# zc402/video-classification

Measured on AMD Instinct MI355X. Metric: clips/sec SlowFast-R50 8x8, 32x224^2 bf16 training step, higher is better.
Workload: dtype bf16

## Files before the change

video-classification_amd/build.py:

```python
import os
import subprocess
from concurrent.futures import ThreadPoolExecutor

HERE = os.path.dirname(os.path.abspath(__file__))
ROOT = os.path.dirname(HERE)
CSRC = os.path.join(HERE, "csrc")
LIB = os.path.join(HERE, "libsfk.so")
SOURCES = ["conv_igemm.hip", "conv_igemm_p8.hip", "conv_halo.hip", "conv_pw.hip", "conv_wgrad.hip", "conv_wgrad_p8.hip", "conv_wgrad_band.hip", "stem_conv.hip", "bn.hip", "bn_tail.hip", "pool_head.hip",
           "optim_misc.hip", "eval_input.hip", "stem2d.hip", "roi_resize.hip", "sgd.hip"]


def _newer(a, b):
    return (not os.path.exists(b)) or os.path.getmtime(a) > os.path.getmtime(b)


def build(force: bool = False, verbose: bool = False) -> str:
    hipcc = os.environ.get("HIPCC", "/opt/rocm/bin/hipcc")
    if not os.path.exists(hipcc):
        hipcc = "hipcc"
    objdir = os.path.join(HERE, "build")
    os.makedirs(objdir, exist_ok=True)
    deps = [os.path.join(CSRC, "sfk_common.h"), os.path.join(CSRC, "conv_igemm_epi.h"), os.path.join(CSRC, "conv_wgrad_common.h"), os.path.join(CSRC, "conv_wgrad_band_acc.inc"), os.path.join(ROOT, "include", "sfk.h"),
            os.path.join(ROOT, "include", "sfk_stem2d.h"), os.path.join(ROOT, "include", "sfk_u8stem.h"),
            os.path.join(ROOT, "include", "sfk_v2.h")]
    flags = ["--offload-arch=gfx950", "-O3", "-fPIC", "-std=c++17", "-I" + os.path.join(ROOT, "include"), "-I" + CSRC]
    flags += os.environ.get("SFK_EXTRA_FLAGS", "").split()

    def compile_one(src):
        s = os.path.join(CSRC, src)
        o = os.path.join(objdir, src.replace(".hip", ".o"))
        if force or _newer(s, o) or any(_newer(d, o) for d in deps):
            cmd = [hipcc] + flags + ["-c", s, "-o", o]
            if verbose:
                print(" ".join(cmd))
            subprocess.run(cmd, check=True)
            return o, True
        return o, False

    with ThreadPoolExecutor(max_workers=min(4, len(SOURCES))) as ex:
        res = list(ex.map(compile_one, SOURCES))
    objs = [o for o, _ in res]
    if force or any(ch for _, ch in res) or not os.path.exists(LIB):
        subprocess.run([hipcc, "--offload-arch=gfx950", "-shared", "-fPIC", "-o", LIB] + objs, check=True)
    return LIB


if __name__ == "__main__":
    print(build(force="--force" in os.sys.argv, verbose=True))
```

video-classification_amd/csrc/conv_halo.hip:

```cpp
#include "conv_igemm_epi.h"

namespace sfk_igemm {

typedef __attribute__((address_space(3))) void lds_void_h_t;

struct HaloTaps { int widx[9]; };

template <int EPI>
__global__ __launch_bounds__(256, 1) void conv_halo_kernel(const ConvK k, const HaloTaps ht, const int nbands, const int bands_per_frame) {
  using T = bf16_t;
  constexpr int C = 64, W = 56;
  constexpr int R = 4;
  constexpr int PW = 64;
  constexpr int PB = C * 2;
  constexpr int ROWBYTES = PW * PB;
  constexpr int BAND = (R + 2) * ROWBYTES;
  constexpr int NBI = BAND / 1024 / 4;
  constexpr int NK = 18;
  constexpr int BM = R * W;
  constexpr int RED0 = 2 * BAND;
  constexpr uint32_t FAR = 0x80000000u;
  __shared__ __attribute__((aligned(16))) char smem[RED0 + 2048];

  const int tid = threadIdx.x, lane = tid & 63;
  const int wave = __builtin_amdgcn_readfirstlane(tid >> 6);
  const int wm = wave & 1, wn = wave >> 1;
  const int l15 = lane & 15, g4 = lane >> 4;
  const int b0 = (gridDim.x & 7) == 0 ? (int)((blockIdx.x & 7) * (gridDim.x >> 3) + (blockIdx.x >> 3)) : (int)blockIdx.x;
  if (b0 >= nbands) return;
  const __amdgpu_buffer_rsrc_t xrs = sfk_make_rsrc(k.x, k.xbytes);
  auto fsw = [](int q) { return ((q >> 1) & 3) << 1; };

  uint32_t bsrc[NBI];
#pragma unroll
  for (int ii = 0; ii < NBI; ++ii) {
    const int qd = (wave * NBI + ii) * 8 + (lane >> 3);
    const int ri = qd / PW, wi = qd % PW;
    const int ls = (lane & 7) ^ fsw(qd);
    bsrc[ii] = (wi >= 1 && wi <= W) ? (uint32_t)((ri * W + wi) * k.xld * 2 + k.xoff * 2 + ls * 16) : FAR;
  }
  int nb_base = 0, nb_r0 = 0;
  auto band_begin = [&](const int b_) __attribute__((always_inline)) {
    const int b = b_ < nbands ? b_ : 0;
    const int fr = b / bands_per_frame;
    nb_r0 = (b - fr * bands_per_frame) * R;
    nb_base = ((fr * k.xh + nb_r0) * W - W - 1) * k.xld * 2;
  };
  auto issue_band = [&](const int buf, const int first, const int count) __attribute__((always_inline)) {
    char* dst = smem + buf * BAND + wave * NBI * 1024;
#pragma unroll
    for (int ii = first; ii < first + count; ++ii) {
      const int ri = (wave * NBI + ii) * 8 / PW;
      const bool rok = (unsigned)(nb_r0 - 1 + ri) < (unsigned)k.xh;
      const uint32_t vo = (rok && bsrc[ii] != FAR) ? (uint32_t)((int)bsrc[ii] + nb_base) : FAR;
      __builtin_amdgcn_raw_ptr_buffer_load_lds(xrs, (lds_void_h_t*)(dst + ii * 1024), 16, (int)vo, 0, 0, 0);
    }
  };
  band_begin(b0);
  issue_band(0, 0, NBI);

  bf16x8 wreg[2][NK];
  {
    const bf16_t* wp = static_cast<const bf16_t*>(k.w);
#pragma unroll
    for (int i = 0; i < 2; ++i) {
      const int co = wn * 32 + 16 * i + l15;
#pragma unroll
      for (int n = 0; n < NK; ++n)
        wreg[i][n] = *reinterpret_cast<const bf16x8*>(wp + ((int64_t)co * k.wtaps + ht.widx[n >> 1]) * k.cin + 32 * (n & 1) + 8 * g4);
    }
  }
  uint32_t xa[2][3][7][2];
#pragma unroll
  for (int j = 0; j < 7; ++j) {
    const int p = wm * 112 + 16 * j + l15;
    const int q0 = (p / W) * PW + (p % W) + 1;
#pragma unroll
    for (int dw = 0; dw < 3; ++dw) {
      const int q = q0 + dw - 1;
#pragma unroll
      for (int sk = 0; sk < 2; ++sk)
#pragma unroll
        for (int bf = 0; bf < 2; ++bf) xa[bf][dw][j][sk] = (uint32_t)(bf * BAND + q * PB + (((4 * sk + g4) ^ fsw(q)) << 4));
    }
  }

  f32x4 acc[2][7];
  bf16x8 xfr[2][7];
  constexpr int BPK = 2, BKS = NBI / BPK;
  static_assert(NBI % BPK == 0 && BKS <= NK, "band pieces");

  auto band_body = [&](const int buf, const int b, const bool first) __attribute__((always_inline)) {
    auto rd_x = [&](const int set, const int n) __attribute__((always_inline)) {
      const int tap = n >> 1, dh = tap / 3 - 1, dw = tap % 3;
#pragma unroll
      for (int j = 0; j < 7; ++j) xfr[set][j] = *reinterpret_cast<const bf16x8*>(smem + xa[buf][dw][j][n & 1] + (dh + 1) * ROWBYTES);
    };
#pragma unroll
    for (int i = 0; i < 2; ++i)
#pragma unroll
      for (int j = 0; j < 7; ++j) acc[i][j] = f32x4{0.f, 0.f, 0.f, 0.f};
    band_begin(b + (int)gridDim.x);
    if (first) asm volatile("s_waitcnt vmcnt(0)" ::: "memory");
    __builtin_amdgcn_s_barrier();
    asm volatile("" ::: "memory");
    rd_x(0, 0);
#pragma unroll
    for (int n = 0; n < NK; ++n) {
      if (n < BKS) issue_band(buf ^ 1, n * BPK, BPK);
      if (n + 1 < NK) rd_x((n + 1) & 1, n + 1);
#pragma unroll
      for (int i = 0; i < 2; ++i)
#pragma unroll
        for (int j = 0; j < 7; ++j)
          asm volatile("v_mfma_f32_16x16x32_bf16 %0, %1, %2, %0" : "+a"(acc[i][j]) : "a"(wreg[i][n]), "v"(xfr[n & 1][j]));
    }
    asm volatile("s_waitcnt vmcnt(0)\n\ts_nop 15\n\ts_nop 7" ::: "memory");
    if (k.stats) {
      float* red = reinterpret_cast<float*>(smem + RED0);
#pragma unroll
      for (int i = 0; i < 2; ++i)
#pragma unroll
        for (int r = 0; r < 4; ++r) {
          float s1 = 0.f, s2 = 0.f;
#pragma unroll
          for (int j = 0; j < 7; ++j) {
            const float v = acc[i][j][r];
            s1 += v;
            s2 += v * v;
          }
          s1 = row16_sum(s1);
          s2 = row16_sum(s2);
          if (l15 == 15) {
            const int col = wn * 32 + 16 * i + 4 * g4 + r;
            red[(wm * 64 + col) * 2 + 0] = s1;
            red[(wm * 64 + col) * 2 + 1] = s2;
          }
        }
      __builtin_amdgcn_s_waitcnt(0xC07F);
      __builtin_amdgcn_s_barrier();
      asm volatile("" ::: "memory");
      if (tid < 64) {
        float* o = k.stats + ((int64_t)b * k.cout + tid) * 2;
        o[0] = red[tid * 2 + 0] + red[(64 + tid) * 2 + 0];
        o[1] = red[tid * 2 + 1] + red[(64 + tid) * 2 + 1];
      }
    }
    ConvK ks = k;
    ks.stats = nullptr;
    epilogue_plain<T, EPI, 7, 2, BM, C, 2, 2, true>(ks, acc, nullptr, b, 0, wm, wn, lane, tid);
  };
  for (int b = b0;;) {
    band_body(0, b, b == b0);
    b += gridDim.x;
    if (b >= nbands) break;
    band_body(1, b, false);
    b += gridDim.x;
    if (b >= nbands) break;
  }
}

__attribute__((visibility("hidden"))) bool halo_ok(const sfk_conv_desc* d) {
  if (!sfk_tune().igemm_halo || d->x.dtype != SFK_BF16) return false;
  if (d->cin != 64 || d->cout != 64 || d->x.w != 56) return false;
  if (d->x.h % 4 != 0 || d->x.t != d->y.t || d->x.h != d->y.h || d->x.w != d->y.w || d->rt != d->y.t || d->rh != d->y.h || d->rw != d->y.w)
    return false;
  for (int a = 0; a < 3; ++a)
    if (d->gs[a] != 1 || d->os[a] != 1 || d->oo[a] != 0) return false;
  if (d->ntaps != 9) return false;
  int seen = 0;
  for (int i = 0; i < 9; ++i) {
    if (d->taps[i].dt != 0 || d->taps[i].dh < -1 || d->taps[i].dh > 1 || d->taps[i].dw < -1 || d->taps[i].dw > 1) return false;
    seen |= 1 << ((d->taps[i].dh + 1) * 3 + d->taps[i].dw + 1);
  }
  if (seen != 0x1FF) return false;
  if (d->ep.scale || d->ep.shift || d->bnb.partials || d->out_relu_bits || d->accumulate) return false;
  if ((d->y.ld % 8) || (d->y.c_off % 8) || !sfk_tune().igemm_wide_store) return false;
  return sfk_fmap_bytes(&d->x) < 0x7FF00000ll;
}

__attribute__((visibility("hidden"))) int halo_mtiles(const sfk_conv_desc* d) { return d->x.n * d->x.t * (d->x.h / 4); }

__attribute__((visibility("hidden"))) int launch_halo(const ConvK& k, const sfk_conv_desc* d, hipStream_t s) {
  const int bpf = d->x.h / 4, nbands = d->x.n * d->x.t * bpf;
  const int grid = nbands < 256 ? nbands : 256;
  HaloTaps ht;
  for (int i = 0; i < 9; ++i) ht.widx[(d->taps[i].dh + 1) * 3 + d->taps[i].dw + 1] = d->taps[i].widx;
  hipLaunchKernelGGL((conv_halo_kernel<0>), dim3((unsigned)grid), dim3(256), 0, s, k, ht, nbands, bpf);
  SFK_CHECK_LAUNCH();
  return SFK_OK;
}

}
```

video-classification_amd/csrc/conv_igemm.hip:

```cpp

#include "conv_igemm_epi.h"

using namespace sfk_igemm;

namespace sfk_igemm {
__attribute__((visibility("hidden"))) int launch_p8(const ConvK& k, int bms, dim3 grid, hipStream_t s);
__attribute__((visibility("hidden"))) bool halo_ok(const sfk_conv_desc* d);
__attribute__((visibility("hidden"))) int halo_mtiles(const sfk_conv_desc* d);
__attribute__((visibility("hidden"))) int launch_halo(const ConvK& k, const sfk_conv_desc* d, hipStream_t s);
}

namespace {

template <typename T, int BM, int BN, int WM, int WN, bool SHORTK, int EPI = 0>
__global__ __launch_bounds__(256, (sizeof(T) == 2 ? 3 : 1)) void conv_igemm_kernel(const ConvK k) {
  using TL = Tile<T>;
  constexpr int VEC = TL::VEC, SEGS = TL::SEGS, ROWB = TL::ROWB;
  constexpr int FM = BM / WM / 16, FN = BN / WN / 16;
  constexpr int RPI = 256 / SEGS;
  constexpr int XL = BM / RPI;
  constexpr int WL = (BN + RPI - 1) / RPI;
  constexpr int BUF = (BM + BN) * ROWB;
  static_assert(WM * WN == 4 && BM % RPI == 0, "tile shape");
  __shared__ __attribute__((aligned(16))) char smem[2 * BUF];
  __shared__ sfk_tap s_taps[SFK_MAX_TAPS + 1];
  __shared__ int s_xdelta[SFK_MAX_TAPS + 1];
  __shared__ int s_woff[SFK_MAX_TAPS + 1];
  if (threadIdx.x <= SFK_MAX_TAPS) {
    sfk_tap t = k.taps[threadIdx.x < SFK_MAX_TAPS ? threadIdx.x : 0];
    if ((int)threadIdx.x >= k.ntaps) { t.dt = -128; t.dh = 0; t.dw = 0; t.widx = 0; }
    s_taps[threadIdx.x] = t;
    s_xdelta[threadIdx.x] = (((int)t.dt * k.xh + (int)t.dh) * k.xw + (int)t.dw) * k.xld * (int)sizeof(T);
    s_woff[threadIdx.x] = (int)t.widx * k.cin * (int)sizeof(T);
  }
  __syncthreads();

  const int tid = threadIdx.x, lane = tid & 63, wave = tid >> 6;
  const int wm = wave % WM, wn = wave / WM;
  const int l15 = lane & 15, g = lane >> 4;

  int mt, nt;
  {
    const int nblk = gridDim.x, b = blockIdx.x;
    const int q = nblk >> 3, r = nblk & 7, xcd = b & 7;
    const int logical = (xcd < r ? xcd * (q + 1) : r * (q + 1) + (xcd - r) * q) + (b >> 3);
    nt = logical % k.ntiles;
    mt = logical / k.ntiles;
  }

  const int seg = tid % SEGS, row0 = tid / SEGS;
  int xtb[XL], xhb[XL], xwb[XL];
  uint32_t xbase[XL];
#pragma unroll
  for (int i = 0; i < XL; ++i) {
    const int m = mt * BM + row0 + i * RPI;
    uint32_t q1, rw_, q2, rh_, n_, rt_;
    k.drw.divmod((uint32_t)m, q1, rw_);
    k.drh.divmod(q1, q2, rh_);
    k.drt.divmod(q2, n_, rt_);
    xtb[i] = (m < k.M) ? (int)rt_ * k.gst : -(1 << 28);
    xhb[i] = (int)rh_ * k.gsh;
    xwb[i] = (int)rw_ * k.gsw;
    xbase[i] = (uint32_t)((((((int64_t)n_ * k.xt + (int)rt_ * k.gst) * k.xh + xhb[i]) * k.xw + xwb[i]) * k.xld + k.xoff) *
                          (int64_t)sizeof(T));
  }
  uint32_t wbase[WL];
#pragma unroll
  for (int i = 0; i < WL; ++i) {
    const int r = row0 + i * RPI;
    const int co = nt * BN + r;
    wbase[i] = (r < BN && co < k.cout) ? (uint32_t)(co * k.wtaps * k.cin) * (uint32_t)sizeof(T) : SFK_OOB;
  }
  const __amdgpu_buffer_rsrc_t xrs = sfk_make_rsrc(k.x, k.xbytes);
  const __amdgpu_buffer_rsrc_t wrs = sfk_make_rsrc(k.w, k.wbytes);

  struct Stage { uint4 x[XL]; uint4 w[WL]; };
  auto gload = [&](int step, Stage& st) {
    const uint32_t q = (uint32_t)(step * SEGS + seg);
    uint32_t tap, cseg;
    k.dspt.divmod(q, tap, cseg);
    const bool cok = tap < (uint32_t)k.ntaps;
    const int ti_ = cok ? (int)tap : SFK_MAX_TAPS;
    const sfk_tap tp = s_taps[ti_];
    const uint32_t xd = (uint32_t)(s_xdelta[ti_] + (int)cseg * 16);
    const uint32_t wd = (uint32_t)(s_woff[ti_] + (int)cseg * 16);
#pragma unroll
    for (int i = 0; i < XL; ++i) {
      const int ti = xtb[i] + tp.dt, hi = xhb[i] + tp.dh, wi = xwb[i] + tp.dw;
      const bool ok = cok && (unsigned)ti < (unsigned)k.xt && (unsigned)hi < (unsigned)k.xh &&
                      (unsigned)wi < (unsigned)k.xw;
      st.x[i] = sfk_buffer_load16(xrs, ok ? xbase[i] + xd : SFK_OOB);
    }
#pragma unroll
    for (int i = 0; i < WL; ++i)
      st.w[i] = sfk_buffer_load16(wrs, (cok && wbase[i] != SFK_OOB) ? wbase[i] + wd : SFK_OOB);
  };
  auto lstore = [&](int buf, const Stage& st) {
    char* xs = smem + buf * BUF;
    char* ws = xs + BM * ROWB;
#pragma unroll
    for (int i = 0; i < XL; ++i) *reinterpret_cast<uint4*>(xs + TL::off(row0 + i * RPI, seg)) = st.x[i];
#pragma unroll
    for (int i = 0; i < WL; ++i) {
      const int r = row0 + i * RPI;
      if ((BN % RPI == 0) || r < BN) *reinterpret_cast<uint4*>(ws + TL::off(r, seg)) = st.w[i];
    }
  };

  f32x4 acc[FN][FM];
#pragma unroll
  for (int i = 0; i < FN; ++i)
#pragma unroll
    for (int j = 0; j < FM; ++j) acc[i][j] = f32x4{0.f, 0.f, 0.f, 0.f};

  auto compute = [&](int buf) {
    const char* xs = smem + buf * BUF;
    const char* ws = xs + BM * ROWB;
    typename TL::frag a[FN], b[FM];
#pragma unroll
    for (int i = 0; i < FN; ++i) a[i] = TL::load(ws, wn * (BN / WN) + 16 * i + l15, g);
#pragma unroll
    for (int j = 0; j < FM; ++j) b[j] = TL::load(xs, wm * (BM / WM) + 16 * j + l15, g);
#pragma unroll
    for (int i = 0; i < FN; ++i)
#pragma unroll
      for (int j = 0; j < FM; ++j) TL::mma(acc[i][j], a[i], b[j]);
  };

  Stage r0, r1;
  if constexpr (SHORTK) {
    gload(0, r0);
    lstore(0, r0);
    if (k.KC > 1) gload(1, r1);
    __syncthreads();
    int it = 0;
    for (; it + 3 < k.KC; it += 2) {
      gload(it + 2, r0);
      compute(0);
      lstore(1, r1);
      __syncthreads();
      gload(it + 3, r1);
      compute(1);
      lstore(0, r0);
      __syncthreads();
    }
    const int rem = k.KC - it;
    if (rem == 1) {
      compute(0);
    } else if (rem == 2) {
      compute(0);
      lstore(1, r1);
      __syncthreads();
      compute(1);
    } else {
      gload(it + 2, r0);
      compute(0);
      lstore(1, r1);
      __syncthreads();
      compute(1);
      lstore(0, r0);
      __syncthreads();
      compute(0);
// ... 305 lines not shown
      (d->rw - 1) * d->os[2] + d->oo[2] >= d->y.w)
    return SFK_ERR_INVALID;
  if ((int64_t)d->x.n * d->rt * d->rh * d->rw >= (1ll << 31)) return SFK_ERR_UNSUPPORTED;
  if (!sfk_fmap_vec_ok(&d->x)) return SFK_ERR_UNSUPPORTED;
  if ((d->y.c % 4) || (d->y.ld % 4) || (d->y.c_off % 4) || (((uintptr_t)d->y.ptr) & 15)) return SFK_ERR_UNSUPPORTED;
  if (((uintptr_t)d->w) & 15) return SFK_ERR_UNSUPPORTED;
  const bool bnb_bits = d->bnb.partials && !d->bnb.y_bn.ptr;
  if (d->out_relu_bits) {
    if (d->bnb.partials && !bnb_bits) return SFK_ERR_INVALID;
    if (!relu_out_ok(d)) return SFK_ERR_UNSUPPORTED;
  }
  if (ep_on(d)) {
    const sfk_conv_epilogue& e = d->ep;
    if (d->stats || d->bnb.partials || d->out_relu_bits) return SFK_ERR_INVALID;
    if ((e.relu_bits && !e.relu) || (e.res_scale && !e.res.ptr) || (e.res_shift && !e.res.ptr)) return SFK_ERR_INVALID;
    if (e.res.ptr && (!sfk_fmap_ok(&e.res) || e.res.n != d->y.n || e.res.t != d->y.t || e.res.h != d->y.h ||
                      e.res.w != d->y.w || e.res.c != d->y.c || e.res.dtype != d->y.dtype))
      return SFK_ERR_INVALID;
    if (!lin_out_of(d)) return SFK_ERR_UNSUPPORTED;
    if ((((uintptr_t)e.scale) | ((uintptr_t)e.shift) | ((uintptr_t)e.res_scale) | ((uintptr_t)e.res_shift)) & 15)
      return SFK_ERR_UNSUPPORTED;
    if (d->x.dtype == SFK_BF16) {
      if (d->cout > 16 ? !bnb_ok(d) : (e.res.ptr || e.relu)) return SFK_ERR_UNSUPPORTED;
    }
    if (e.res.ptr && !sfk_fmap_vec_ok(&e.res)) return SFK_ERR_UNSUPPORTED;
    if (sfk_fmap_bytes(&d->y) >= (1ll << 32) - 64 || (e.res.ptr && sfk_fmap_bytes(&e.res) >= (1ll << 32) - 64))
      return SFK_ERR_UNSUPPORTED;
  }
  if (d->bnb.partials) {
    if (sfk_fmap_bytes(&d->y) >= (1ll << 32) - 64) return SFK_ERR_UNSUPPORTED;
    if (d->bnb.y_bn.ptr && sfk_fmap_ok(&d->bnb.y_bn) && sfk_fmap_bytes(&d->bnb.y_bn) >= (1ll << 32) - 64) return SFK_ERR_UNSUPPORTED;
    if (d->bnb.mask_src.ptr && sfk_fmap_ok(&d->bnb.mask_src) && sfk_fmap_bytes(&d->bnb.mask_src) >= (1ll << 32) - 64) return SFK_ERR_UNSUPPORTED;
  }
  if (bnb_bits) {
    if (!d->out_relu_bits || d->stats || d->bnb.mask_src.ptr) return SFK_ERR_INVALID;
    if (!bnb_ok(d) || !lin_out_of(d)) return SFK_ERR_UNSUPPORTED;
  } else if (d->bnb.partials) {
    const sfk_bn_bwd_fuse& b = d->bnb;
    if (d->stats || !sfk_fmap_ok(&b.y_bn) || !b.mean || !b.invstd) return SFK_ERR_INVALID;
    if (b.y_bn.n != d->y.n || b.y_bn.t != d->y.t || b.y_bn.h != d->y.h || b.y_bn.w != d->y.w || b.y_bn.c != d->y.c ||
        b.y_bn.dtype != d->y.dtype)
      return SFK_ERR_INVALID;
    if (b.mask_src.ptr && (!sfk_fmap_ok(&b.mask_src) || b.mask_src.n != d->y.n || b.mask_src.t != d->y.t ||
                           b.mask_src.h != d->y.h || b.mask_src.w != d->y.w || b.mask_src.c != d->y.c ||
                           b.mask_src.dtype != d->y.dtype))
      return SFK_ERR_INVALID;
    if (!b.mask_src.ptr && b.relu && (!b.scale || !b.shift)) return SFK_ERR_INVALID;
    if (!bnb_ok(d)) return SFK_ERR_UNSUPPORTED;
    if (!sfk_fmap_vec_ok(&b.y_bn) || (b.mask_src.ptr && !sfk_fmap_vec_ok(&b.mask_src))) return SFK_ERR_UNSUPPORTED;
  }
  const int64_t esz = d->x.dtype == SFK_BF16 ? 2 : 4;
  if (sfk_fmap_bytes(&d->x) >= (1ll << 32) - 64 || (int64_t)d->cout * d->wtaps * d->cin * esz >= (1ll << 32) - 64)
    return SFK_ERR_UNSUPPORTED;
  return SFK_OK;
}

int launch_dma(const ConvK& k, int bm, dim3 grid, hipStream_t s, int bn = 128) {
  if (bn == 256) {
    if (bm == 224) hipLaunchKernelGGL((conv_igemm_dma_kernel<256, 256, 2, 4, 0, 224>), grid, dim3(512), 0, s, k);
    else hipLaunchKernelGGL((conv_igemm_dma_kernel<256, 256, 4, 2>), grid, dim3(512), 0, s, k);
    SFK_CHECK_LAUNCH();
    return SFK_OK;
  }
  if (k.bn_parts) {
    if (k.bn_y == nullptr) hipLaunchKernelGGL((conv_igemm_dma_kernel<128, 128, 2, 2, 5>), grid, dim3(256), 0, s, k);
    else if (k.bn_mask) hipLaunchKernelGGL((conv_igemm_dma_kernel<128, 128, 2, 2, 7>), grid, dim3(256), 0, s, k);
    else if (k.accumulate) hipLaunchKernelGGL((conv_igemm_dma_kernel<128, 128, 2, 2, 6>), grid, dim3(256), 0, s, k);
    else hipLaunchKernelGGL((conv_igemm_dma_kernel<128, 128, 2, 2, 1>), grid, dim3(256), 0, s, k);
    SFK_CHECK_LAUNCH();
    return SFK_OK;
  }
  if (k.ep_on) {
    if (bm == 256) hipLaunchKernelGGL((conv_igemm_dma_kernel<256, 128, 4, 2, 3>), grid, dim3(512), 0, s, k);
    else if (k.ep_res) hipLaunchKernelGGL((conv_igemm_dma_kernel<128, 128, 2, 2, 4>), grid, dim3(256), 0, s, k);
    else hipLaunchKernelGGL((conv_igemm_dma_kernel<128, 128, 2, 2, 3>), grid, dim3(256), 0, s, k);
    SFK_CHECK_LAUNCH();
    return SFK_OK;
  }
  if (k.obits) {
    if (bm == 256) hipLaunchKernelGGL((conv_igemm_dma_kernel<256, 128, 4, 2, 2>), grid, dim3(512), 0, s, k);
    else hipLaunchKernelGGL((conv_igemm_dma_kernel<128, 128, 2, 2, 2>), grid, dim3(256), 0, s, k);
    SFK_CHECK_LAUNCH();
    return SFK_OK;
  }
  if (bm == 256) hipLaunchKernelGGL((conv_igemm_dma_kernel<256, 128, 4, 2>), grid, dim3(512), 0, s, k);
  else hipLaunchKernelGGL((conv_igemm_dma_kernel<128, 128, 2, 2>), grid, dim3(256), 0, s, k);
  SFK_CHECK_LAUNCH();
  return SFK_OK;
}

template <typename T>
int launch(const sfk_conv_desc* d, hipStream_t s) {
  ConvK k;
  k.x = d->x.ptr; k.y = d->y.ptr; k.w = d->w; k.stats = d->stats;
  k.xt = d->x.t; k.xh = d->x.h; k.xw = d->x.w; k.xld = d->x.ld; k.xoff = d->x.c_off;
  k.yt = d->y.t; k.yh = d->y.h; k.yw = d->y.w; k.yld = d->y.ld; k.yoff = d->y.c_off;
  k.M = d->x.n * d->rt * d->rh * d->rw;
  k.drw.set(d->rw); k.drh.set(d->rh); k.drt.set(d->rt);
  k.gst = d->gs[0]; k.gsh = d->gs[1]; k.gsw = d->gs[2];
  k.ost = d->os[0]; k.osh = d->os[1]; k.osw = d->os[2];
  k.oot = d->oo[0]; k.ooh = d->oo[1]; k.oow = d->oo[2];
  k.cin = d->cin; k.cout = d->cout; k.wtaps = d->wtaps; k.ntaps = d->ntaps;
  const int vec = sfk_vec_of(d->x.dtype), segs = BK / vec;
  k.dspt.set(d->cin / vec);
  k.dkct.set(d->cin / 32 > 0 ? d->cin / 32 : 1);
  k.dk64.set(d->ntaps);
  k.KC = (d->ntaps * (d->cin / vec) + segs - 1) / segs;
  k.accumulate = d->accumulate;
  k.obits = d->out_relu_bits;
  k.bn_parts = d->bnb.partials;
  k.bn_y = nullptr; k.bn_mask = nullptr;
  if (k.bn_parts) {
    k.bn_y = d->bnb.y_bn.ptr; k.bn_yld = d->bnb.y_bn.ld; k.bn_yoff = d->bnb.y_bn.c_off;
    k.bn_mask = d->bnb.mask_src.ptr; k.bn_mld = d->bnb.mask_src.ld; k.bn_moff = d->bnb.mask_src.c_off;
    k.bn_relu = d->bnb.relu;
    k.bn_mean = d->bnb.mean; k.bn_invstd = d->bnb.invstd; k.bn_scale = d->bnb.scale; k.bn_shift = d->bnb.shift;
  }
  k.ep_on = ep_on(d) ? 1 : 0;
  k.ep_scale = d->ep.scale; k.ep_shift = d->ep.shift; k.ep_rscale = d->ep.res_scale; k.ep_rshift = d->ep.res_shift;
  k.ep_res = d->ep.res.ptr; k.ep_rld = d->ep.res.ld; k.ep_roff = d->ep.res.c_off;
  k.ep_relu = d->ep.relu; k.ep_bits = d->ep.relu_bits;
  k.ybytes = (uint32_t)sfk_fmap_bytes(&d->y);
  k.ybig = sfk_fmap_bytes(&d->y) >= (1ll << 32) - 64 ? 1 : 0;
  k.ep_rbytes = d->ep.res.ptr ? (uint32_t)sfk_fmap_bytes(&d->ep.res) : 0u;
  k.bn_ybytes = (k.bn_parts && d->bnb.y_bn.ptr) ? (uint32_t)sfk_fmap_bytes(&d->bnb.y_bn) : 0u;
  k.bn_mbytes = (k.bn_parts && d->bnb.mask_src.ptr) ? (uint32_t)sfk_fmap_bytes(&d->bnb.mask_src) : 0u;
  k.obits_bytes = d->out_relu_bits ? (uint32_t)(sfk_fmap_pixels(&d->y) * (d->cout / sfk_vec_of(d->x.dtype))) : 0u;
  k.kshort = sfk_tune().igemm_short_k;
  k.lin_out = lin_out_of(d);
  const int wide_ok = sfk_tune().igemm_wide_store;
  k.wide_store = (wide_ok || k.obits) && (d->cout % 8) == 0 && (d->y.ld % 8) == 0 && (d->y.c_off % 8) == 0;
  k.xbytes = (uint32_t)sfk_fmap_bytes(&d->x);
  k.wbytes = (uint32_t)((int64_t)d->cout * d->wtaps * d->cin * (d->x.dtype == SFK_BF16 ? 2 : 4));
  for (int i = 0; i < SFK_MAX_TAPS; ++i) k.taps[i] = d->taps[i < d->ntaps ? i : 0];
  if constexpr (sizeof(T) == 2) {
    if (k.ep_on && (d->ep.res.ptr || d->ep.relu) && !d->accumulate && sfk_tune().igemm_pw_stream && d->ntaps == 1 &&
        d->taps[0].dt == 0 && d->taps[0].dh == 0 && d->taps[0].dw == 0 && d->gs[0] == 1 && d->gs[1] == 1 && d->gs[2] == 1 &&
        k.lin_out && d->x.t == d->y.t && d->x.h == d->y.h && d->x.w == d->y.w) {
      const int r = sfk_conv_pw_fused(d, s);
      if (r != SFK_ERR_UNSUPPORTED) return r;
    }
    if (pw_dgrad_rows(d) > 0) return sfk_conv_pw_dgrad(d, s);
    if (pw_plain_route(d)) {
      const int r = sfk_conv_pw_fused(d, s);
      if (r != SFK_ERR_UNSUPPORTED) return r;
    }
  }
  if constexpr (sizeof(T) == 2) {
    if (halo_ok(d)) {
      k.mtiles = halo_mtiles(d);
      k.ntiles = 1;
      return launch_halo(k, d, s);
    }
  }
  const TileSel ts = pick_tile(d);
  k.mtiles = (k.M + ts.bm - 1) / ts.bm;
  k.ntiles = (d->cout + ts.bn - 1) / ts.bn;
  const dim3 grid((unsigned)(k.mtiles * k.ntiles)), block(256);
  if (ts.p8) return launch_p8(k, ts.bm, dim3((unsigned)(k.mtiles * k.ntiles)), s);
  if (ts.dma) return launch_dma(k, ts.bm, grid, s, ts.bn);
  if (k.bn_parts) {
    if constexpr (sizeof(T) == 2) {
      if (k.bn_y == nullptr) {
        if (ts.bn == 128) hipLaunchKernelGGL((conv_igemm_kernel<T, 128, 128, 2, 2, false, 5>), grid, block, 0, s, k);
        else if (ts.bn == 64) hipLaunchKernelGGL((conv_igemm_kernel<T, 256, 64, 4, 1, false, 5>), grid, block, 0, s, k);
        else hipLaunchKernelGGL((conv_igemm_kernel<T, 256, 32, 4, 1, false, 5>), grid, block, 0, s, k);
      } else if (k.bn_mask) {
        if (ts.bn == 128) hipLaunchKernelGGL((conv_igemm_kernel<T, 128, 128, 2, 2, false, 7>), grid, block, 0, s, k);
        else if (ts.bn == 64) hipLaunchKernelGGL((conv_igemm_kernel<T, 256, 64, 4, 1, false, 7>), grid, block, 0, s, k);
        else hipLaunchKernelGGL((conv_igemm_kernel<T, 256, 32, 4, 1, false, 7>), grid, block, 0, s, k);
      } else if (k.accumulate) {
        if (ts.bn == 128) hipLaunchKernelGGL((conv_igemm_kernel<T, 128, 128, 2, 2, false, 6>), grid, block, 0, s, k);
        else if (ts.bn == 64) hipLaunchKernelGGL((conv_igemm_kernel<T, 256, 64, 4, 1, false, 6>), grid, block, 0, s, k);
        else hipLaunchKernelGGL((conv_igemm_kernel<T, 256, 32, 4, 1, false, 6>), grid, block, 0, s, k);
      } else if (ts.bn == 128) hipLaunchKernelGGL((conv_igemm_kernel<T, 128, 128, 2, 2, false, 1>), grid, block, 0, s, k);
      else if (ts.bn == 64) hipLaunchKernelGGL((conv_igemm_kernel<T, 256, 64, 4, 1, false, 1>), grid, block, 0, s, k);
      else hipLaunchKernelGGL((conv_igemm_kernel<T, 256, 32, 4, 1, false, 1>), grid, block, 0, s, k);
      SFK_CHECK_LAUNCH();
      return SFK_OK;
    }
    return SFK_ERR_UNSUPPORTED;
  }
  if (k.ep_on) {
    if (ts.bn == 128) hipLaunchKernelGGL((conv_igemm_kernel<T, 128, 128, 2, 2, false, 3>), grid, block, 0, s, k);
    else if (ts.bn == 64) hipLaunchKernelGGL((conv_igemm_kernel<T, 256, 64, 4, 1, false, 3>), grid, block, 0, s, k);
    else if (ts.bn == 32) hipLaunchKernelGGL((conv_igemm_kernel<T, 256, 32, 4, 1, false, 3>), grid, block, 0, s, k);
    else hipLaunchKernelGGL((conv_igemm_kernel<T, 256, 16, 4, 1, false, 3>), grid, block, 0, s, k);
    SFK_CHECK_LAUNCH();
    return SFK_OK;
  }
  if (k.obits) {
    if (ts.bn == 128) hipLaunchKernelGGL((conv_igemm_kernel<T, 128, 128, 2, 2, false, 2>), grid, block, 0, s, k);
    else if (ts.bn == 64) hipLaunchKernelGGL((conv_igemm_kernel<T, 256, 64, 4, 1, false, 2>), grid, block, 0, s, k);
    else if (ts.bn == 32) hipLaunchKernelGGL((conv_igemm_kernel<T, 256, 32, 4, 1, false, 2>), grid, block, 0, s, k);
    else if (sizeof(T) == 4) hipLaunchKernelGGL((conv_igemm_kernel<T, 256, 16, 4, 1, false, 2>), grid, block, 0, s, k);
    else return SFK_ERR_UNSUPPORTED;
    SFK_CHECK_LAUNCH();
    return SFK_OK;
  }
  if (k.KC <= k.kshort && ts.bn <= 32) {
    if (ts.bn == 32) hipLaunchKernelGGL((conv_igemm_kernel<T, 256, 32, 4, 1, true>), grid, block, 0, s, k);
    else hipLaunchKernelGGL((conv_igemm_kernel<T, 256, 16, 4, 1, true>), grid, block, 0, s, k);
  } else {
    if (ts.bn == 128) hipLaunchKernelGGL((conv_igemm_kernel<T, 128, 128, 2, 2, false>), grid, block, 0, s, k);
    else if (ts.bn == 64) hipLaunchKernelGGL((conv_igemm_kernel<T, 256, 64, 4, 1, false>), grid, block, 0, s, k);
    else if (ts.bn == 32) hipLaunchKernelGGL((conv_igemm_kernel<T, 256, 32, 4, 1, false>), grid, block, 0, s, k);
    else hipLaunchKernelGGL((conv_igemm_kernel<T, 256, 16, 4, 1, false>), grid, block, 0, s, k);
  }
  SFK_CHECK_LAUNCH();
  return SFK_OK;
}

}

extern "C" int sfk_conv_igemm_mtiles(const sfk_conv_desc* d) {
  const int st = validate(d);
  if (st != SFK_OK) return st;
  const int rows = pw_dgrad_rows(d);
  if (rows > 0) return rows;
  if (halo_ok(d)) return halo_mtiles(d);
  const int64_t M = (int64_t)d->x.n * d->rt * d->rh * d->rw;
  const int bm = pick_tile(d).bm;
  return (int)((M + bm - 1) / bm);
}

extern "C" int sfk_conv_relu_out_supported(const sfk_conv_desc* d) {
  if (!d || d->struct_size != sizeof(sfk_conv_desc)) return 0;
  sfk_conv_desc c = *d;
  c.out_relu_bits = nullptr;
  if (validate(&c) != SFK_OK) return 0;
  return relu_out_ok(d) ? 1 : 0;
}

extern "C" int sfk_conv_igemm_family(const sfk_conv_desc* d) {
  if (validate(d) != SFK_OK) return -1;
  if (d->x.dtype == SFK_BF16) {
    if (ep_on(d) && (d->ep.res.ptr || d->ep.relu) && !d->accumulate && sfk_tune().igemm_pw_stream && d->ntaps == 1 &&
        d->taps[0].dt == 0 && d->taps[0].dh == 0 && d->taps[0].dw == 0 && d->gs[0] == 1 && d->gs[1] == 1 && d->gs[2] == 1 &&
        lin_out_of(d) && d->x.t == d->y.t && d->x.h == d->y.h && d->x.w == d->y.w && d->cin <= 128 &&
        ((d->cout == 32 || d->cout == 64 || d->cout == 128) ? d->cin <= 32 : (d->cout == 256 ? (d->cin > 32 && d->cin <= 64) : (d->cout == 512 && d->cin > 96))))
      return 3;
    if (pw_dgrad_rows(d) > 0) return 3;
    if (pw_plain_route(d)) return 3;
  }
  if (halo_ok(d)) return 5;
  const TileSel ts = pick_tile(d);
  return ts.p8 ? 4 : (ts.dma ? 1 : 0);
}

extern "C" int sfk_conv_epilogue_supported(const sfk_conv_desc* d) {
  return (d && ep_on(d) && validate(d) == SFK_OK) ? 1 : 0;
}

extern "C" int sfk_conv_bnb_supported(const sfk_conv_desc* d) {
  if (!d || d->struct_size != sizeof(sfk_conv_desc)) return 0;
  sfk_conv_desc c = *d;
  c.bnb.partials = nullptr;
  if (validate(&c) != SFK_OK) return 0;
  return bnb_ok(d) ? 1 : 0;
}

extern "C" int sfk_conv_igemm(const sfk_conv_desc* d, sfk_stream_t stream) {
  const int st = validate(d);
  if (st != SFK_OK) return st;
  hipStream_t s = static_cast<hipStream_t>(stream);
  return d->x.dtype == SFK_BF16 ? launch<bf16_t>(d, s) : launch<float>(d, s);
}
```

video-classification_amd/csrc/optim_misc.hip:

```cpp
#include <string.h>

#include "sfk_common.h"

namespace {

__global__ void adam_step_inc_kernel(int64_t* step) { step[0] += 1; }

template <typename S>
__global__ __launch_bounds__(256) void adam_kernel(float* __restrict__ p, const float* __restrict__ g,
                                                   float* __restrict__ m, float* __restrict__ v, int64_t count,
                                                   float lr, float b1, float b2, float eps, float gscale,
                                                   const int64_t* step, S* __restrict__ shadow) {
  __shared__ float bc[2];
  if (threadIdx.x == 0) {
    const double t = (double)step[0];
    bc[0] = (float)(1.0 - pow((double)b1, t));
    bc[1] = (float)(1.0 - pow((double)b2, t));
  }
  __syncthreads();
  const float step_size = lr / bc[0];
  const float inv_sqrt_bc2 = 1.f / sqrtf(bc[1]);
  for (int64_t i = ((int64_t)blockIdx.x * 256 + threadIdx.x) * 4; i < count; i += (int64_t)gridDim.x * 1024) {
    if (i + 3 < count) {
      float4 pv = *reinterpret_cast<float4*>(p + i);
// ... 18 lines not shown
#pragma unroll
        for (int j = 0; j < 4; ++j) shadow[i + j] = (S)pp[j];
      }
    } else {
      for (int64_t e = i; e < count; ++e) {
        const float gj = g[e] * gscale;
        m[e] = b1 * m[e] + (1.f - b1) * gj;
        v[e] = b2 * v[e] + (1.f - b2) * gj * gj;
        p[e] -= step_size * m[e] / (sqrtf(v[e]) * inv_sqrt_bc2 + eps);
        if (shadow) shadow[e] = (S)p[e];
      }
    }
  }
}

template <typename S, typename D>
__global__ __launch_bounds__(256) void cast_kernel(const S* __restrict__ src, D* __restrict__ dst, int64_t count) {
  for (int64_t i = (int64_t)blockIdx.x * 256 + threadIdx.x; i < count; i += (int64_t)gridDim.x * 256)
    dst[i] = (D)(float)src[i];
}

template <typename S, typename D>
__global__ __launch_bounds__(256) void filter_transpose_kernel(const S* __restrict__ src, D* __restrict__ dst,
                                                               int cout, int wtaps, int cin) {
  const int64_t total = (int64_t)cout * wtaps * cin;
  for (int64_t i = (int64_t)blockIdx.x * 256 + threadIdx.x; i < total; i += (int64_t)gridDim.x * 256) {
    const int co = (int)(i % cout);
    const int64_t r = i / cout;
    const int wi = (int)(r % wtaps);
    const int ci = (int)(r / wtaps);
    dst[i] = (D)(float)src[((int64_t)co * wtaps + wi) * cin + ci];
  }
}

template <typename D>
__global__ __launch_bounds__(256) void filter_refresh_kernel(const float* __restrict__ master, D* __restrict__ s,
                                                             D* __restrict__ st, const sfk_filter_ent* __restrict__ table,
                                                             int n) {
  __shared__ float tile[32][33];
  int lo = 0, hi = n - 1;
  const int b = blockIdx.x;
  while (lo < hi) {
    const int mid = (lo + hi + 1) >> 1;
    if (table[mid].first_block <= b) lo = mid; else hi = mid - 1;
  }
  const sfk_filter_ent e = table[lo];
  const int tiles_ci = (e.cin + 31) / 32;
  int lb = b - e.first_block;
  const int tap = lb % e.wtaps;
  lb /= e.wtaps;
  const int ci0 = (lb % tiles_ci) * 32, co0 = (lb / tiles_ci) * 32;
  const int tx = threadIdx.x & 31, ty = threadIdx.x >> 5;
#pragma unroll
  for (int i = 0; i < 4; ++i) {
    const int co = co0 + ty + 8 * i, ci = ci0 + tx;
    float v = 0.f;
    if (co < e.cout && ci < e.cin) {
      const int64_t idx = e.off + ((int64_t)co * e.wtaps + tap) * e.cin + ci;
      v = master[idx];
      if (s) s[idx] = (D)v;
    }
    tile[ty + 8 * i][tx] = v;
  }
  if (!st || !e.transpose) return;
  __syncthreads();
#pragma unroll
  for (int i = 0; i < 4; ++i) {
    const int ci = ci0 + ty + 8 * i, co = co0 + tx;
    if (co < e.cout && ci < e.cin) st[e.off + ((int64_t)ci * e.wtaps + tap) * e.cout + co] = (D)tile[tx][ty + 8 * i];
  }
}

inline unsigned grid_for(int64_t total, int per_thread = 1) {
  int64_t b = (total + 256ll * per_thread - 1) / (256ll * per_thread);
  if (b > 16384) b = 16384;
  if (b < 1) b = 1;
  return (unsigned)b;
}

}

extern "C" int sfk_adam(float* p, const float* g, float* m, float* v, int64_t count, float lr, float beta1,
                        float beta2, float eps, float grad_scale, int64_t* step, void* shadow,
                        int32_t shadow_dtype, sfk_stream_t stream) {
  if (!p || !g || !m || !v || !step || count <= 0) return SFK_ERR_INVALID;
  if ((((uintptr_t)p) | ((uintptr_t)g) | ((uintptr_t)m) | ((uintptr_t)v)) & 15) return SFK_ERR_UNSUPPORTED;
  hipStream_t s = static_cast<hipStream_t>(stream);
  hipLaunchKernelGGL(adam_step_inc_kernel, dim3(1), dim3(1), 0, s, step);
  const dim3 grid(grid_for(count, 4)), blk(256);
  if (shadow && shadow_dtype == SFK_BF16)
    hipLaunchKernelGGL(adam_kernel<bf16_t>, grid, blk, 0, s, p, g, m, v, count, lr, beta1, beta2, eps, grad_scale, step, static_cast<bf16_t*>(shadow));
  else
    hipLaunchKernelGGL(adam_kernel<float>, grid, blk, 0, s, p, g, m, v, count, lr, beta1, beta2, eps, grad_scale, step, static_cast<float*>(shadow));
  SFK_CHECK_LAUNCH();
  return SFK_OK;
}


static inline bool dtype_ok(int d) { return d == SFK_F32 || d == SFK_BF16; }

extern "C" int sfk_filter_transpose(const void* src, int32_t src_dtype, void* dst, int32_t dst_dtype, int32_t cout,
                                    int32_t wtaps, int32_t cin, sfk_stream_t stream) {
  if (!src || !dst || cout <= 0 || wtaps <= 0 || cin <= 0 || !dtype_ok(src_dtype) || !dtype_ok(dst_dtype))
    return SFK_ERR_INVALID;
  hipStream_t s = static_cast<hipStream_t>(stream);
  const int64_t total = (int64_t)cout * wtaps * cin;
  if (src_dtype == SFK_F32 && dst_dtype == SFK_F32)
    hipLaunchKernelGGL((filter_transpose_kernel<float, float>), dim3(grid_for(total)), dim3(256), 0, s, (const float*)src, (float*)dst, cout, wtaps, cin);
  else if (src_dtype == SFK_F32 && dst_dtype == SFK_BF16)
    hipLaunchKernelGGL((filter_transpose_kernel<float, bf16_t>), dim3(grid_for(total)), dim3(256), 0, s, (const float*)src, (bf16_t*)dst, cout, wtaps, cin);
  else if (src_dtype == SFK_BF16 && dst_dtype == SFK_F32)
    hipLaunchKernelGGL((filter_transpose_kernel<bf16_t, float>), dim3(grid_for(total)), dim3(256), 0, s, (const bf16_t*)src, (float*)dst, cout, wtaps, cin);
  else
    hipLaunchKernelGGL((filter_transpose_kernel<bf16_t, bf16_t>), dim3(grid_for(total)), dim3(256), 0, s, (const bf16_t*)src, (bf16_t*)dst, cout, wtaps, cin);
  SFK_CHECK_LAUNCH();
  return SFK_OK;
}

extern "C" int sfk_filter_refresh(const float* master, void* s, void* st, int32_t dtype, const sfk_filter_ent* table,
                                  int32_t n_layers, int32_t total_blocks, sfk_stream_t stream) {
  if (!master || (!s && !st) || !table || n_layers <= 0 || total_blocks <= 0 || !dtype_ok(dtype)) return SFK_ERR_INVALID;
  hipStream_t hs = static_cast<hipStream_t>(stream);
  if (dtype == SFK_BF16)
    hipLaunchKernelGGL((filter_refresh_kernel<bf16_t>), dim3((unsigned)total_blocks), dim3(256), 0, hs, master, (bf16_t*)s, (bf16_t*)st, table, n_layers);
  else
    hipLaunchKernelGGL((filter_refresh_kernel<float>), dim3((unsigned)total_blocks), dim3(256), 0, hs, master, (float*)s, (float*)st, table, n_layers);
  SFK_CHECK_LAUNCH();
  return SFK_OK;
}

extern "C" int sfk_cast(const void* src, int32_t src_dtype, void* dst, int32_t dst_dtype, int64_t count,
                        sfk_stream_t stream) {
  if (!src || !dst || count <= 0 || !dtype_ok(src_dtype) || !dtype_ok(dst_dtype)) return SFK_ERR_INVALID;
  hipStream_t s = static_cast<hipStream_t>(stream);
  if (src_dtype == SFK_F32 && dst_dtype == SFK_F32)
    hipLaunchKernelGGL((cast_kernel<float, float>), dim3(grid_for(count, 4)), dim3(256), 0, s, (const float*)src, (float*)dst, count);
  else if (src_dtype == SFK_F32 && dst_dtype == SFK_BF16)
    hipLaunchKernelGGL((cast_kernel<float, bf16_t>), dim3(grid_for(count, 4)), dim3(256), 0, s, (const float*)src, (bf16_t*)dst, count);
  else if (src_dtype == SFK_BF16 && dst_dtype == SFK_F32)
    hipLaunchKernelGGL((cast_kernel<bf16_t, float>), dim3(grid_for(count, 4)), dim3(256), 0, s, (const bf16_t*)src, (float*)dst, count);
  else
    hipLaunchKernelGGL((cast_kernel<bf16_t, bf16_t>), dim3(grid_for(count, 4)), dim3(256), 0, s, (const bf16_t*)src, (bf16_t*)dst, count);
  SFK_CHECK_LAUNCH();
  return SFK_OK;
}

extern "C" int sfk_fill_zero(void* p, size_t bytes, sfk_stream_t stream) {
  if (!p) return SFK_ERR_INVALID;
  if (bytes == 0) return SFK_OK;
  return hipMemsetAsync(p, 0, bytes, static_cast<hipStream_t>(stream)) == hipSuccess ? SFK_OK : SFK_ERR_LAUNCH;
}

namespace {
constexpr sfk_tuning kDefaults = {(uint32_t)sizeof(sfk_tuning), 5, 0, 1, 192, 256, 1, 7, 1024, 0, 48, 150, 1, 1ll << 20, 3, 512, 1, 16, 1, 3, 3};
sfk_tuning g_tuning = kDefaults;
bool g_tuning_set = false;
}
const sfk_tuning& sfk_tune() { return g_tuning; }

extern "C" int sfk_default_tuning(sfk_tuning* out) {
  if (!out || out->struct_size != sizeof(sfk_tuning)) return SFK_ERR_INVALID;
  *out = kDefaults;
  return SFK_OK;
}

extern "C" int sfk_get_tuning(sfk_tuning* out) {
  if (!out || out->struct_size != sizeof(sfk_tuning)) return SFK_ERR_INVALID;
  *out = g_tuning;
  return SFK_OK;
}

extern "C" int sfk_init(const sfk_tuning* t) {
  sfk_tuning want = kDefaults;
  if (t) {
    if (t->struct_size != sizeof(sfk_tuning)) return SFK_ERR_INVALID;
    want = *t;
  }
  if (want.bn_parts < 1 || want.wgrad_target_8w < 1 || want.wgrad_target_4w < 1 || want.pool_blocks < 1 ||
      want.igemm_short_k < 0)
    return SFK_ERR_INVALID;
  if (g_tuning_set) return memcmp(&want, &g_tuning, sizeof(want)) == 0 ? SFK_OK : SFK_ERR_INVALID;
  g_tuning = want;
  g_tuning_set = true;
  return SFK_OK;
}

extern "C" int sfk_abi_version(void) { return SFK_ABI_VERSION; }

extern "C" const char* sfk_status_string(int status) {
  switch (status) {
    case SFK_OK: return "ok";
    case SFK_ERR_INVALID: return "invalid argument";
    case SFK_ERR_UNSUPPORTED: return "unsupported shape or alignment";
    case SFK_ERR_LAUNCH: return "kernel launch failed";
    default: return "unknown status";
  }
}
```

Before: 1168.

## Add narrow-channel halo conv kernel for 8- and 16-channel 3x3 convs

Adds a new halo-band implicit-GEMM kernel for small-channel 3x3 spatial convs (8ch at width 56, 16ch at width 28), which in SlowFast are the fast pathway. It packs several taps into one MFMA K-dimension and stages 14-row bands through LDS with double buffering. It also fuses the BN stats reduction into the kernel. The igemm_halo tuning field becomes a bitmask and defaults to enabling both narrow variants, routing these convs away from the generic igemm path, which wastes most of its tile on tiny channel counts. The kernel covers only forward-style convs with no epilogue.

```diff
diff --git a/video-classification_amd/build.py b/video-classification_amd/build.py
--- a/video-classification_amd/build.py
+++ b/video-classification_amd/build.py
@@ -6,7 +6,7 @@
 ROOT = os.path.dirname(HERE)
 CSRC = os.path.join(HERE, "csrc")
 LIB = os.path.join(HERE, "libsfk.so")
-SOURCES = ["conv_igemm.hip", "conv_igemm_p8.hip", "conv_halo.hip", "conv_pw.hip", "conv_wgrad.hip", "conv_wgrad_p8.hip", "conv_wgrad_band.hip", "stem_conv.hip", "bn.hip", "bn_tail.hip", "pool_head.hip",
+SOURCES = ["conv_igemm.hip", "conv_igemm_p8.hip", "conv_halo.hip", "conv_halo_narrow.hip", "conv_pw.hip", "conv_wgrad.hip", "conv_wgrad_p8.hip", "conv_wgrad_band.hip", "stem_conv.hip", "bn.hip", "bn_tail.hip", "pool_head.hip",
            "optim_misc.hip", "eval_input.hip", "stem2d.hip", "roi_resize.hip", "sgd.hip"]
 
 
diff --git a/video-classification_amd/csrc/conv_halo.hip b/video-classification_amd/csrc/conv_halo.hip
--- a/video-classification_amd/csrc/conv_halo.hip
+++ b/video-classification_amd/csrc/conv_halo.hip
@@ -161,7 +161,7 @@
 }
 
 __attribute__((visibility("hidden"))) bool halo_ok(const sfk_conv_desc* d) {
-  if (!sfk_tune().igemm_halo || d->x.dtype != SFK_BF16) return false;
+  if (!(sfk_tune().igemm_halo & 1) || d->x.dtype != SFK_BF16) return false;
   if (d->cin != 64 || d->cout != 64 || d->x.w != 56) return false;
   if (d->x.h % 4 != 0 || d->x.t != d->y.t || d->x.h != d->y.h || d->x.w != d->y.w || d->rt != d->y.t || d->rh != d->y.h || d->rw != d->y.w)
     return false;
diff --git a/video-classification_amd/csrc/conv_halo_narrow.hip b/video-classification_amd/csrc/conv_halo_narrow.hip
--- /dev/null
+++ b/video-classification_amd/csrc/conv_halo_narrow.hip
@@ -0,0 +1,215 @@
+#include "conv_igemm_epi.h"
+
+namespace sfk_igemm {
+
+typedef __attribute__((address_space(3))) void lds_void_n_t;
+
+struct NarrowTaps { int widx[9]; };
+
+constexpr int NARROW_R = 14;
+constexpr int NARROW_GRID = 1024;
+
+template <int C, int W>
+__global__ __launch_bounds__(256, 4) void conv_halo_narrow_kernel(const ConvK k, const NarrowTaps ht, const int nbands, const int bands_per_frame) {
+  static_assert(C == 8 || C == 16, "one or two 16-byte planes");
+  constexpr int R = NARROW_R;
+  constexpr int PW = (W + 2 + 7) / 8 * 8;
+  constexpr int NPL = C / 8;
+  constexpr int PLANE = (R + 2) * PW * 16;
+  constexpr int BAND = NPL * PLANE;
+  constexpr int NBI = BAND / 1024 / 4;
+  constexpr int TPS = 4 / NPL;
+  constexpr int NK = (9 + TPS - 1) / TPS;
+  constexpr int BM = R * W;
+  constexpr int NF = (BM + 15) / 16;
+  constexpr int NP = (NF + 1) / 2;
+  constexpr int NPW = (NP + 3) / 4;
+  constexpr int RED0 = 2 * BAND;
+  constexpr uint32_t FAR = 0x80000000u;
+  static_assert(BAND == 16384 && NBI == 4 && (PW & (PW - 1)) == 0 && NBI <= NPW, "band layout");
+  __shared__ __attribute__((aligned(16))) char smem[RED0 + 4 * 16 * 2 * 4];
+
+  const int tid = threadIdx.x, lane = tid & 63;
+  const int wave = __builtin_amdgcn_readfirstlane(tid >> 6);
+  const int l15 = lane & 15, g4 = lane >> 4;
+  const int b0 = (gridDim.x & 7) == 0 ? (int)((blockIdx.x & 7) * (gridDim.x >> 3) + (blockIdx.x >> 3)) : (int)blockIdx.x;
+  if (b0 >= nbands) return;
+  const __amdgpu_buffer_rsrc_t xrs = sfk_make_rsrc(k.x, k.xbytes);
+
+  uint32_t bsrc[NBI];
+  int brow[NBI];
+#pragma unroll
+  for (int ii = 0; ii < NBI; ++ii) {
+    const int rec = (wave * NBI + ii) * 64 + lane;
+    const int pl = rec / (PLANE / 16), qd = rec % (PLANE / 16);
+    const int ri = qd / PW, wi = qd % PW;
+    brow[ii] = ri;
+    bsrc[ii] = (wi >= 1 && wi <= W) ? (uint32_t)((ri * W + wi) * k.xld * 2 + k.xoff * 2 + pl * 16) : FAR;
+  }
+  int nb_base = 0, nb_r0 = 0;
+  auto band_begin = [&](const int b_) __attribute__((always_inline)) {
+    const int b = b_ < nbands ? b_ : 0;
+    const int fr = b / bands_per_frame;
+    nb_r0 = (b - fr * bands_per_frame) * R;
+    nb_base = ((fr * k.xh + nb_r0) * W - W - 1) * k.xld * 2;
+  };
+  auto issue_band = [&](const int buf, const int ii) __attribute__((always_inline)) {
+    char* dst = smem + buf * BAND + (wave * NBI + ii) * 1024;
+    const bool rok = (unsigned)(nb_r0 - 1 + brow[ii]) < (unsigned)k.xh;
+    const uint32_t vo = (rok && bsrc[ii] != FAR) ? (uint32_t)((int)bsrc[ii] + nb_base) : FAR;
+    __builtin_amdgcn_raw_ptr_buffer_load_lds(xrs, (lds_void_n_t*)dst, 16, (int)vo, 0, 0, 0);
+  };
+  band_begin(b0);
+#pragma unroll
+  for (int ii = 0; ii < NBI; ++ii) issue_band(0, ii);
+
+  const int tsub = C == 8 ? g4 : (g4 >> 1);
+  const int half = C == 8 ? 0 : (g4 & 1);
+  bf16x8 zero8;
+#pragma unroll
+  for (int e = 0; e < 8; ++e) zero8[e] = (bf16_t)0.f;
+  bf16x8 wreg[NK];
+  uint32_t toff[NK];
+  const bool tok_last = (NK - 1) * TPS + tsub < 9;
+  static_assert((NK - 1) * TPS <= 9, "padding slots in the last k-step only");
+  {
+    const bf16_t* wp = static_cast<const bf16_t*>(k.w);
+#pragma unroll
+    for (int n = 0; n < NK; ++n) {
+      const int ts = n * TPS + tsub;
+      const bool tok = ts < 9;
+      const int tc = tok ? ts : 0;
+      toff[n] = (uint32_t)(((tc / 3) * PW + (tc % 3)) * 16 + half * PLANE);
+      wreg[n] = zero8;
+      if (tok && l15 < C) wreg[n] = *reinterpret_cast<const bf16x8*>(wp + ((int64_t)l15 * k.wtaps + ht.widx[tc]) * k.cin + 8 * half);
+    }
+  }
+  uint32_t xq[NPW][2];
+#pragma unroll
+  for (int i = 0; i < NPW; ++i)
+#pragma unroll
+    for (int f = 0; f < 2; ++f) {
+      const int p = ((wave + 4 * i) * 2 + f) * 16 + l15;
+      xq[i][f] = p < BM ? (uint32_t)(((p / W) * PW + (p % W)) * 16) : 0u;
+    }
+  const int sch = 8 * (g4 >> 1);
+  bf16_t* const yp = static_cast<bf16_t*>(k.y);
+
+  auto band_body = [&](const int buf, const int b, const bool first) __attribute__((always_inline)) {
+    band_begin(b + (int)gridDim.x);
+    if (first) asm volatile("s_waitcnt vmcnt(0)" ::: "memory");
+    __builtin_amdgcn_s_barrier();
+    asm volatile("" ::: "memory");
+    const char* img = smem + buf * BAND;
+    bf16x8 outv[NPW];
+    float s1[4] = {0.f, 0.f, 0.f, 0.f}, s2[4] = {0.f, 0.f, 0.f, 0.f};
+#pragma unroll
+    for (int i = 0; i < NPW; ++i) {
+      if (i < NBI) issue_band(buf ^ 1, i);
+      if (wave + 4 * i < NP) {
+        f32x4 acc[2] = {f32x4{0.f, 0.f, 0.f, 0.f}, f32x4{0.f, 0.f, 0.f, 0.f}};
+        bf16x8 xfr[2][NK];
+#pragma unroll
+        for (int n = 0; n < NK; ++n)
+#pragma unroll
+          for (int f = 0; f < 2; ++f) {
+            xfr[f][n] = *reinterpret_cast<const bf16x8*>(img + xq[i][f] + toff[n]);
+            if (n == NK - 1 && !tok_last) xfr[f][n] = zero8;
+          }
+#pragma unroll
+        for (int n = 0; n < NK; ++n)
+#pragma unroll
+          for (int f = 0; f < 2; ++f) acc[f] = __builtin_amdgcn_mfma_f32_16x16x32_bf16(wreg[n], xfr[f][n], acc[f], 0, 0, 0);
+        float v[8];
+#pragma unroll
+        for (int f = 0; f < 2; ++f) {
+          const bool pok = ((wave + 4 * i) * 2 + f) * 16 + l15 < BM;
+#pragma unroll
+          for (int r = 0; r < 4; ++r) {
+            const float a = pok ? acc[f][r] : 0.f;
+            v[4 * f + r] = a;
+            s1[r] += a;
+            s2[r] += a * a;
+          }
+        }
+#pragma unroll
+        for (int e = 0; e < 4; ++e) swap16(v[e], v[4 + e]);
+#pragma unroll
+        for (int e = 0; e < 8; ++e) outv[i][e] = (bf16_t)v[e];
+      }
+    }
+    asm volatile("s_waitcnt vmcnt(0)" ::: "memory");
+    if (k.stats) {
+      float* red = reinterpret_cast<float*>(smem + RED0);
+#pragma unroll
+      for (int r = 0; r < 4; ++r) {
+        const float a = row16_sum(s1[r]), c = row16_sum(s2[r]);
+        if (l15 == 15) {
+          red[(wave * 16 + 4 * g4 + r) * 2 + 0] = a;
+          red[(wave * 16 + 4 * g4 + r) * 2 + 1] = c;
+        }
+      }
+      __builtin_amdgcn_s_waitcnt(0xC07F);
+      __builtin_amdgcn_s_barrier();
+      asm volatile("" ::: "memory");
+      if (tid < C) {
+        float* o = k.stats + ((int64_t)b * k.cout + tid) * 2;
+        o[0] = ((red[tid * 2 + 0] + red[(16 + tid) * 2 + 0]) + red[(32 + tid) * 2 + 0]) + red[(48 + tid) * 2 + 0];
+        o[1] = ((red[tid * 2 + 1] + red[(16 + tid) * 2 + 1]) + red[(32 + tid) * 2 + 1]) + red[(48 + tid) * 2 + 1];
+      }
+    }
+#pragma unroll
+    for (int i = 0; i < NPW; ++i) {
+      const int p = ((wave + 4 * i) * 2 + (g4 & 1)) * 16 + l15;
+      if (wave + 4 * i < NP && p < BM && sch < C)
+        *reinterpret_cast<bf16x8*>(yp + ((int64_t)b * BM + p) * k.yld + k.yoff + sch) = outv[i];
+    }
+  };
+  for (int b = b0;;) {
+    band_body(0, b, b == b0);
+    b += gridDim.x;
+    if (b >= nbands) break;
+    band_body(1, b, false);
+    b += gridDim.x;
+    if (b >= nbands) break;
+  }
+}
+
+__attribute__((visibility("hidden"))) int halo_narrow_ok(const sfk_conv_desc* d) {
+  const int bits = sfk_tune().igemm_halo;
+  if (!(bits & 6) || d->x.dtype != SFK_BF16 || d->y.dtype != SFK_BF16) return 0;
+  int c = 0;
+  if ((bits & 2) && d->cin == 8 && d->cout == 8 && d->x.w == 56) c = 8;
+  if ((bits & 4) && d->cin == 16 && d->cout == 16 && d->x.w == 28) c = 16;
+  if (!c) return 0;
+  if (d->x.h % NARROW_R != 0 || d->x.t != d->y.t || d->x.h != d->y.h || d->x.w != d->y.w || d->rt != d->y.t || d->rh != d->y.h || d->rw != d->y.w)
+    return 0;
+  for (int a = 0; a < 3; ++a)
+    if (d->gs[a] != 1 || d->os[a] != 1 || d->oo[a] != 0) return 0;
+  if (d->ntaps != 9) return 0;
+  int seen = 0;
+  for (int i = 0; i < 9; ++i) {
+    if (d->taps[i].dt != 0 || d->taps[i].dh < -1 || d->taps[i].dh > 1 || d->taps[i].dw < -1 || d->taps[i].dw > 1) return 0;
+    seen |= 1 << ((d->taps[i].dh + 1) * 3 + d->taps[i].dw + 1);
+  }
+  if (seen != 0x1FF) return 0;
+  if (d->ep.scale || d->ep.shift || d->bnb.partials || d->out_relu_bits || d->accumulate) return 0;
+  if ((d->x.ld % 8) || (d->x.c_off % 8) || (d->y.ld % 8) || (d->y.c_off % 8) || !sfk_tune().igemm_wide_store) return 0;
+  if (sfk_fmap_bytes(&d->x) >= 0x7FF00000ll || sfk_fmap_bytes(&d->y) >= 0x7FF00000ll) return 0;
+  return c;
+}
+
+__attribute__((visibility("hidden"))) int halo_narrow_mtiles(const sfk_conv_desc* d) { return d->x.n * d->x.t * (d->x.h / NARROW_R); }
+
+__attribute__((visibility("hidden"))) int launch_halo_narrow(const ConvK& k, const sfk_conv_desc* d, hipStream_t s) {
+  const int bpf = d->x.h / NARROW_R, nbands = d->x.n * d->x.t * bpf;
+  const int grid = nbands < NARROW_GRID ? nbands : NARROW_GRID;
+  NarrowTaps ht;
+  for (int i = 0; i < 9; ++i) ht.widx[(d->taps[i].dh + 1) * 3 + d->taps[i].dw + 1] = d->taps[i].widx;
+  if (d->cin == 8) hipLaunchKernelGGL((conv_halo_narrow_kernel<8, 56>), dim3((unsigned)grid), dim3(256), 0, s, k, ht, nbands, bpf);
+  else hipLaunchKernelGGL((conv_halo_narrow_kernel<16, 28>), dim3((unsigned)grid), dim3(256), 0, s, k, ht, nbands, bpf);
+  SFK_CHECK_LAUNCH();
+  return SFK_OK;
+}
+
+}
diff --git a/video-classification_amd/csrc/conv_igemm.hip b/video-classification_amd/csrc/conv_igemm.hip
--- a/video-classification_amd/csrc/conv_igemm.hip
+++ b/video-classification_amd/csrc/conv_igemm.hip
@@ -8,6 +8,9 @@
 __attribute__((visibility("hidden"))) bool halo_ok(const sfk_conv_desc* d);
 __attribute__((visibility("hidden"))) int halo_mtiles(const sfk_conv_desc* d);
 __attribute__((visibility("hidden"))) int launch_halo(const ConvK& k, const sfk_conv_desc* d, hipStream_t s);
+__attribute__((visibility("hidden"))) int halo_narrow_ok(const sfk_conv_desc* d);
+__attribute__((visibility("hidden"))) int halo_narrow_mtiles(const sfk_conv_desc* d);
+__attribute__((visibility("hidden"))) int launch_halo_narrow(const ConvK& k, const sfk_conv_desc* d, hipStream_t s);
 }
 
 namespace {
@@ -619,6 +622,11 @@
       k.ntiles = 1;
       return launch_halo(k, d, s);
     }
+    if (halo_narrow_ok(d)) {
+      k.mtiles = halo_narrow_mtiles(d);
+      k.ntiles = 1;
+      return launch_halo_narrow(k, d, s);
+    }
   }
   const TileSel ts = pick_tile(d);
   k.mtiles = (k.M + ts.bm - 1) / ts.bm;
@@ -686,6 +694,7 @@
   const int rows = pw_dgrad_rows(d);
   if (rows > 0) return rows;
   if (halo_ok(d)) return halo_mtiles(d);
+  if (halo_narrow_ok(d)) return halo_narrow_mtiles(d);
   const int64_t M = (int64_t)d->x.n * d->rt * d->rh * d->rw;
   const int bm = pick_tile(d).bm;
   return (int)((M + bm - 1) / bm);
@@ -710,7 +719,7 @@
     if (pw_dgrad_rows(d) > 0) return 3;
     if (pw_plain_route(d)) return 3;
   }
-  if (halo_ok(d)) return 5;
+  if (halo_ok(d) || halo_narrow_ok(d)) return 5;
   const TileSel ts = pick_tile(d);
   return ts.p8 ? 4 : (ts.dma ? 1 : 0);
 }
diff --git a/video-classification_amd/csrc/optim_misc.hip b/video-classification_amd/csrc/optim_misc.hip
--- a/video-classification_amd/csrc/optim_misc.hip
+++ b/video-classification_amd/csrc/optim_misc.hip
@@ -194,7 +194,7 @@
 }
 
 namespace {
-constexpr sfk_tuning kDefaults = {(uint32_t)sizeof(sfk_tuning), 5, 0, 1, 192, 256, 1, 7, 1024, 0, 48, 150, 1, 1ll << 20, 3, 512, 1, 16, 1, 3, 3};
+constexpr sfk_tuning kDefaults = {(uint32_t)sizeof(sfk_tuning), 5, 0, 1, 192, 256, 1, 7, 1024, 0, 48, 150, 1, 1ll << 20, 3, 512, 1, 16, 7, 3, 3};
 sfk_tuning g_tuning = kDefaults;
 bool g_tuning_set = false;
 }
```

Result: no change. 1176, median of 6 (+0.6%).
